# cleinc/bts

Hardware: NVIDIA H100
Metric: training images/sec (352x704, DenseNet-161) (higher is better)
Workload: dtype f32

## Files before the change

bts_b200/csrc/wgmma_tf32.cuh:

```cuda
#pragma once
#include <stdint.h>

namespace tc {

template <int N> struct Wgmma;

template <> struct Wgmma<16> {
    static __device__ __forceinline__ void mma(float (&d)[8], uint64_t a, uint64_t b, uint32_t scale_d) {
        asm volatile(
            "{\n\t.reg .pred p;\n\tsetp.ne.b32 p, %10, 0;\n\t"
            "wgmma.mma_async.sync.aligned.m64n16k8.f32.tf32.tf32 {%0, %1, %2, %3, %4, %5, %6, %7}, %8, %9, p, 1, 1;\n\t}"
            : "+f"(d[0]), "+f"(d[1]), "+f"(d[2]), "+f"(d[3]), "+f"(d[4]), "+f"(d[5]), "+f"(d[6]), "+f"(d[7])
            : "l"(a), "l"(b), "r"(scale_d));
    }
    static __device__ __forceinline__ void mma_rs(float (&d)[8], const uint32_t (&a)[4], uint64_t b, uint32_t scale_d) {
        asm volatile(
            "{\n\t.reg .pred p;\n\tsetp.ne.b32 p, %13, 0;\n\t"
            "wgmma.mma_async.sync.aligned.m64n16k8.f32.tf32.tf32 {%0, %1, %2, %3, %4, %5, %6, %7}, {%8, %9, %10, %11}, %12, p, 1, 1;\n\t}"
            : "+f"(d[0]), "+f"(d[1]), "+f"(d[2]), "+f"(d[3]), "+f"(d[4]), "+f"(d[5]), "+f"(d[6]), "+f"(d[7])
            : "r"(a[0]), "r"(a[1]), "r"(a[2]), "r"(a[3]), "l"(b), "r"(scale_d));
    }
};

template <> struct Wgmma<32> {
    static __device__ __forceinline__ void mma(float (&d)[16], uint64_t a, uint64_t b, uint32_t scale_d) {
        asm volatile(
            "{\n\t.reg .pred p;\n\tsetp.ne.b32 p, %18, 0;\n\t"
            "wgmma.mma_async.sync.aligned.m64n32k8.f32.tf32.tf32 {%0, %1, %2, %3, %4, %5, %6, %7, %8, %9, %10, %11, %12, %13, %14, %15}, %16, %17, p, 1, 1;\n\t}"
            : "+f"(d[0]), "+f"(d[1]), "+f"(d[2]), "+f"(d[3]), "+f"(d[4]), "+f"(d[5]), "+f"(d[6]), "+f"(d[7]), "+f"(d[8]), "+f"(d[9]), "+f"(d[10]), "+f"(d[11]), "+f"(d[12]), "+f"(d[13]), "+f"(d[14]), "+f"(d[15])
            : "l"(a), "l"(b), "r"(scale_d));
    }
    static __device__ __forceinline__ void mma_rs(float (&d)[16], const uint32_t (&a)[4], uint64_t b, uint32_t scale_d) {
        asm volatile(
            "{\n\t.reg .pred p;\n\tsetp.ne.b32 p, %21, 0;\n\t"
            "wgmma.mma_async.sync.aligned.m64n32k8.f32.tf32.tf32 {%0, %1, %2, %3, %4, %5, %6, %7, %8, %9, %10, %11, %12, %13, %14, %15}, {%16, %17, %18, %19}, %20, p, 1, 1;\n\t}"
            : "+f"(d[0]), "+f"(d[1]), "+f"(d[2]), "+f"(d[3]), "+f"(d[4]), "+f"(d[5]), "+f"(d[6]), "+f"(d[7]), "+f"(d[8]), "+f"(d[9]), "+f"(d[10]), "+f"(d[11]), "+f"(d[12]), "+f"(d[13]), "+f"(d[14]), "+f"(d[15])
            : "r"(a[0]), "r"(a[1]), "r"(a[2]), "r"(a[3]), "l"(b), "r"(scale_d));
    }
};

template <> struct Wgmma<48> {
    static __device__ __forceinline__ void mma(float (&d)[24], uint64_t a, uint64_t b, uint32_t scale_d) {
        asm volatile(
            "{\n\t.reg .pred p;\n\tsetp.ne.b32 p, %26, 0;\n\t"
            "wgmma.mma_async.sync.aligned.m64n48k8.f32.tf32.tf32 {%0, %1, %2, %3, %4, %5, %6, %7, %8, %9, %10, %11, %12, %13, %14, %15, %16, %17, %18, %19, %20, %21, %22, %23}, %24, %25, p, 1, 1;\n\t}"
            : "+f"(d[0]), "+f"(d[1]), "+f"(d[2]), "+f"(d[3]), "+f"(d[4]), "+f"(d[5]), "+f"(d[6]), "+f"(d[7]), "+f"(d[8]), "+f"(d[9]), "+f"(d[10]), "+f"(d[11]), "+f"(d[12]), "+f"(d[13]), "+f"(d[14]), "+f"(d[15]), "+f"(d[16]), "+f"(d[17]), "+f"(d[18]), "+f"(d[19]), "+f"(d[20]), "+f"(d[21]), "+f"(d[22]), "+f"(d[23])
            : "l"(a), "l"(b), "r"(scale_d));
    }
    static __device__ __forceinline__ void mma_rs(float (&d)[24], const uint32_t (&a)[4], uint64_t b, uint32_t scale_d) {
        asm volatile(
            "{\n\t.reg .pred p;\n\tsetp.ne.b32 p, %29, 0;\n\t"
            "wgmma.mma_async.sync.aligned.m64n48k8.f32.tf32.tf32 {%0, %1, %2, %3, %4, %5, %6, %7, %8, %9, %10, %11, %12, %13, %14, %15, %16, %17, %18, %19, %20, %21, %22, %23}, {%24, %25, %26, %27}, %28, p, 1, 1;\n\t}"
            : "+f"(d[0]), "+f"(d[1]), "+f"(d[2]), "+f"(d[3]), "+f"(d[4]), "+f"(d[5]), "+f"(d[6]), "+f"(d[7]), "+f"(d[8]), "+f"(d[9]), "+f"(d[10]), "+f"(d[11]), "+f"(d[12]), "+f"(d[13]), "+f"(d[14]), "+f"(d[15]), "+f"(d[16]), "+f"(d[17]), "+f"(d[18]), "+f"(d[19]), "+f"(d[20]), "+f"(d[21]), "+f"(d[22]), "+f"(d[23])
            : "r"(a[0]), "r"(a[1]), "r"(a[2]), "r"(a[3]), "l"(b), "r"(scale_d));
    }
};

template <> struct Wgmma<64> {
    static __device__ __forceinline__ void mma(float (&d)[32], uint64_t a, uint64_t b, uint32_t scale_d) {
        asm volatile(
            "{\n\t.reg .pred p;\n\tsetp.ne.b32 p, %34, 0;\n\t"
            "wgmma.mma_async.sync.aligned.m64n64k8.f32.tf32.tf32 {%0, %1, %2, %3, %4, %5, %6, %7, %8, %9, %10, %11, %12, %13, %14, %15, %16, %17, %18, %19, %20, %21, %22, %23, %24, %25, %26, %27, %28, %29, %30, %31}, %32, %33, p, 1, 1;\n\t}"
            : "+f"(d[0]), "+f"(d[1]), "+f"(d[2]), "+f"(d[3]), "+f"(d[4]), "+f"(d[5]), "+f"(d[6]), "+f"(d[7]), "+f"(d[8]), "+f"(d[9]), "+f"(d[10]), "+f"(d[11]), "+f"(d[12]), "+f"(d[13]), "+f"(d[14]), "+f"(d[15]), "+f"(d[16]), "+f"(d[17]), "+f"(d[18]), "+f"(d[19]), "+f"(d[20]), "+f"(d[21]), "+f"(d[22]), "+f"(d[23]), "+f"(d[24]), "+f"(d[25]), "+f"(d[26]), "+f"(d[27]), "+f"(d[28]), "+f"(d[29]), "+f"(d[30]), "+f"(d[31])
            : "l"(a), "l"(b), "r"(scale_d));
    }
    static __device__ __forceinline__ void mma_rs(float (&d)[32], const uint32_t (&a)[4], uint64_t b, uint32_t scale_d) {
        asm volatile(
            "{\n\t.reg .pred p;\n\tsetp.ne.b32 p, %37, 0;\n\t"
            "wgmma.mma_async.sync.aligned.m64n64k8.f32.tf32.tf32 {%0, %1, %2, %3, %4, %5, %6, %7, %8, %9, %10, %11, %12, %13, %14, %15, %16, %17, %18, %19, %20, %21, %22, %23, %24, %25, %26, %27, %28, %29, %30, %31}, {%32, %33, %34, %35}, %36, p, 1, 1;\n\t}"
            : "+f"(d[0]), "+f"(d[1]), "+f"(d[2]), "+f"(d[3]), "+f"(d[4]), "+f"(d[5]), "+f"(d[6]), "+f"(d[7]), "+f"(d[8]), "+f"(d[9]), "+f"(d[10]), "+f"(d[11]), "+f"(d[12]), "+f"(d[13]), "+f"(d[14]), "+f"(d[15]), "+f"(d[16]), "+f"(d[17]), "+f"(d[18]), "+f"(d[19]), "+f"(d[20]), "+f"(d[21]), "+f"(d[22]), "+f"(d[23]), "+f"(d[24]), "+f"(d[25]), "+f"(d[26]), "+f"(d[27]), "+f"(d[28]), "+f"(d[29]), "+f"(d[30]), "+f"(d[31])
            : "r"(a[0]), "r"(a[1]), "r"(a[2]), "r"(a[3]), "l"(b), "r"(scale_d));
    }
};

template <> struct Wgmma<80> {
    static __device__ __forceinline__ void mma(float (&d)[40], uint64_t a, uint64_t b, uint32_t scale_d) {
        asm volatile(
            "{\n\t.reg .pred p;\n\tsetp.ne.b32 p, %42, 0;\n\t"
            "wgmma.mma_async.sync.aligned.m64n80k8.f32.tf32.tf32 {%0, %1, %2, %3, %4, %5, %6, %7, %8, %9, %10, %11, %12, %13, %14, %15, %16, %17, %18, %19, %20, %21, %22, %23, %24, %25, %26, %27, %28, %29, %30, %31, %32, %33, %34, %35, %36, %37, %38, %39}, %40, %41, p, 1, 1;\n\t}"
            : "+f"(d[0]), "+f"(d[1]), "+f"(d[2]), "+f"(d[3]), "+f"(d[4]), "+f"(d[5]), "+f"(d[6]), "+f"(d[7]), "+f"(d[8]), "+f"(d[9]), "+f"(d[10]), "+f"(d[11]), "+f"(d[12]), "+f"(d[13]), "+f"(d[14]), "+f"(d[15]), "+f"(d[16]), "+f"(d[17]), "+f"(d[18]), "+f"(d[19]), "+f"(d[20]), "+f"(d[21]), "+f"(d[22]), "+f"(d[23]), "+f"(d[24]), "+f"(d[25]), "+f"(d[26]), "+f"(d[27]), "+f"(d[28]), "+f"(d[29]), "+f"(d[30]), "+f"(d[31]), "+f"(d[32]), "+f"(d[33]), "+f"(d[34]), "+f"(d[35]), "+f"(d[36]), "+f"(d[37]), "+f"(d[38]), "+f"(d[39])
            : "l"(a), "l"(b), "r"(scale_d));
    }
};

}
```

bts_b200/csrc/wgrad2_tc.cu:

```cuda
#include <cuda.h>

#include <cstring>
#include <type_traits>

#include "tc_common.cuh"

using namespace tc;

namespace {

constexpr int BLOCK_CI = 64;
constexpr int X_CHUNKS = BLOCK_CI / 32;
constexpr int KP = 16;
constexpr uint32_t CORE_SBO = 4 * 128 + 16;
constexpr int A_BYTES = BLOCK_CI / 8 * CORE_SBO;
constexpr int MAX_TAPS = 9;
constexpr int MAX_NT = 144;
constexpr int MAX_STAGES = 4;
constexpr int CONSUMER_THREADS = 256;
constexpr int LOADER_WARP = CONSUMER_THREADS / 32;
constexpr int GROUPS = 3;
constexpr int PRODUCERS = 128 * GROUPS;
constexpr int NUM_THREADS = CONSUMER_THREADS + 32 + PRODUCERS;
constexpr int SMEM_BUDGET = 224 * 1024;
constexpr int MAX_RING = 4;
constexpr int X_RAW_BYTES = KP * BLOCK_CI * 4;

struct W2Params {
    const float *x; long long xs;
    int B, Hs, Ws, up, Cin;
    int KH, KW, pad, dil;
    const float *pre_scale, *pre_shift;
    const float *dy; long long dys;
    int Cout, Hout, Wout, Hin, Win;
    int cg, nb;
    int nchunks;
    float *part;
    int splitK, kb_per_split, KBq;
    int Mq;
    int stages, stage_bytes, precision;
    int ring, slot_bytes, seg_bytes, segw, tox_max, slot_tx;
};

template <int PRE, bool UP, bool VEC, bool TMA>
__global__ void __launch_bounds__(NUM_THREADS, 1) wgrad2_tc_kernel(const W2Params p, const __grid_constant__ CUtensorMap tmx,
                                                                   const __grid_constant__ CUtensorMap tmd) {
    extern __shared__ __align__(1024) uint8_t smem_raw[];
    const uint32_t base = (smem_u32(smem_raw) + 1023u) & ~1023u;
    uint8_t *sm = smem_raw + (base - smem_u32(smem_raw));
    const int taps = p.KH * p.KW;
    const int S = p.stages;
    const uint32_t ring_off = (uint32_t)S * (uint32_t)p.stage_bytes;
    const uint32_t pre_off = ring_off + (TMA ? (uint32_t)p.ring * (uint32_t)p.slot_bytes : 0u);
    float *s_scale = reinterpret_cast<float *>(sm + pre_off);
    float *s_shift = s_scale + BLOCK_CI;
    const uint32_t bar0 = base + pre_off + 2 * BLOCK_CI * 4;
    auto full = [&](int s) { return bar0 + 8u * s; };
    auto empty = [&](int s) { return bar0 + 8u * (MAX_STAGES + s); };
    auto rfull = [&](int j) { return bar0 + 8u * (2 * MAX_STAGES + j); };
    auto rempty = [&](int j) { return bar0 + 8u * (2 * MAX_STAGES + MAX_RING + j); };
    const int warp = threadIdx.x >> 5, lane = threadIdx.x & 31;
    const int ci_tile = blockIdx.x, cgi = blockIdx.y, split = blockIdx.z;
    const int co0 = cgi * p.cg;
    const int ncol = min(p.cg, ((p.Cout - co0 + 15) >> 4) << 4);
    const int nb = p.nb;
    const int n_total = taps * ncol;
    const uint32_t b_half = (uint32_t)p.nchunks * 4u * CORE_SBO;
    const int kb0 = split * p.kb_per_split;
    int kb1 = kb0 + p.kb_per_split;
    if (kb1 > p.KBq) kb1 = p.KBq;
    const int nkb = kb1 > kb0 ? kb1 - kb0 : 0;

    if (threadIdx.x == 0) {
        for (int s = 0; s < MAX_STAGES; ++s) {
            mbar_init(full(s), PRODUCERS);
            mbar_init(empty(s), CONSUMER_THREADS);
        }
        for (int j = 0; j < MAX_RING; ++j) {
            mbar_init(rfull(j), 1);
            mbar_init(rempty(j), PRODUCERS);
        }
        asm volatile("fence.mbarrier_init.release.cluster;" ::: "memory");
    }
    if (PRE >= 2) {
        for (int c = threadIdx.x; c < BLOCK_CI; c += NUM_THREADS) {
            const int ch = ci_tile * BLOCK_CI + c;
            s_scale[c] = ch < p.Cin ? p.pre_scale[ch] : 0.f;
            s_shift[c] = ch < p.Cin ? p.pre_shift[ch] : 0.f;
        }
    }
    for (int i = threadIdx.x; i < S * p.stage_bytes / 16; i += NUM_THREADS) st_shared_v4(base + i * 16, 0.f, 0.f, 0.f, 0.f);
    fence_proxy_async();
    __syncthreads();

    if (warp == LOADER_WARP) {
        if (TMA && lane == 0) {
            if (!UP) tma_prefetch_desc(&tmx);
            tma_prefetch_desc(&tmd);
            int j = 0;
            uint32_t ph = 0;
            for (int it = 0; it < nkb; ++it) {
                mbar_wait(rempty(j), ph ^ 1);
                const uint32_t dst = base + ring_off + (uint32_t)j * (uint32_t)p.slot_bytes;
                const int q0 = (kb0 + it) * KP;
                mbar_arrive_expect_tx(rfull(j), (uint32_t)p.slot_tx);
                uint32_t seg = dst;
                if (!UP) {
                    tma_tile_2d(dst, &tmx, ci_tile * BLOCK_CI, q0, rfull(j));
                    seg += X_RAW_BYTES;
                }
                for (int ky = 0; ky < p.KH; ++ky)
                    tma_tile_2d(seg + (uint32_t)ky * (uint32_t)p.seg_bytes, &tmd, co0,
                                q0 - (ky * p.dil - p.pad) * p.Wout - p.tox_max, rfull(j));
                if (++j == p.ring) { j = 0; ph ^= 1; }
            }
        }
    } else if (warp < LOADER_WARP) {
        const int wg = warp >> 2;
        const int n_half = (n_total + 31) / 32 * 16;
        const int n0 = wg ? n_half : 0, n_mine = wg ? n_total - n_half : n_half;
        auto consume = [&](auto NT) {
            constexpr int N = decltype(NT)::value;
            float acc[N > 0 ? N / 2 : 1];
#pragma unroll
            for (int i = 0; i < (N > 0 ? N / 2 : 1); ++i) acc[i] = 0.f;
            const bool single = p.precision != 0;
            int s = 0;
            uint32_t ph = 0;
            for (int it = 0; it < nkb; ++it) {
                mbar_wait(full(s), ph);
                wgmma_fence();
                const uint32_t a_hi = base + (uint32_t)s * (uint32_t)p.stage_bytes, a_lo = a_hi + A_BYTES;
                const uint32_t b_hi = a_hi + 2 * A_BYTES + (uint32_t)(n0 >> 3) * CORE_SBO, b_lo = b_hi + b_half;
                if constexpr (N > 0) {
#pragma unroll
                    for (int kg = 0; kg < KP / 8; ++kg) {
                        const uint32_t ko = (uint32_t)kg * 256u;
                        const uint64_t dah = make_desc_core(a_hi + ko, 128, CORE_SBO), dal = make_desc_core(a_lo + ko, 128, CORE_SBO);
                        const uint64_t dbh = make_desc_core(b_hi + ko, 128, CORE_SBO), dbl = make_desc_core(b_lo + ko, 128, CORE_SBO);
                        const uint32_t accumulate = (it | kg) != 0;
                        if (single) {
                            Wgmma<N>::mma(acc, dah, dbh, accumulate);
                        } else {
                            Wgmma<N>::mma(acc, dal, dbh, accumulate);
                            Wgmma<N>::mma(acc, dah, dbl, 1);
                            Wgmma<N>::mma(acc, dah, dbh, 1);
                        }
                    }
                }
                wgmma_commit();
                wgmma_wait<0>();
                mbar_arrive(empty(s));
                if (++s == S) { s = 0; ph ^= 1; }
            }
            wgmma_wait<0>();
            wgmma_fence_operands(acc);
            if (N == 0) return;
            const bool ovec = (p.Cout & 1) == 0 && ((((uintptr_t)p.part) & 7) == 0) && ((co0 & 1) == 0);
#pragma unroll
            for (int i = 0; i < 2; ++i) {
                const int ci = ci_tile * BLOCK_CI + (warp & 3) * 16 + (lane >> 2) + 8 * i;
                if (ci >= p.Cin) continue;
#pragma unroll
                for (int j = 0; j < (N > 0 ? N / 8 : 0); ++j) {
                    const int n = n0 + 8 * j + (lane & 3) * 2;
                    if (n >= n0 + n_mine) continue;
                    const int t = n / ncol, cc = n - t * ncol;
                    float *dst = p.part + (((long long)split * taps + t) * p.Cin + ci) * p.Cout + co0 + cc;
                    const float v0 = acc[4 * j + 2 * i], v1 = acc[4 * j + 2 * i + 1];
                    if (ovec && co0 + cc + 1 < p.Cout) {
                        *reinterpret_cast<float2 *>(dst) = make_float2(v0, v1);
                    } else {
                        if (co0 + cc < p.Cout) dst[0] = v0;
                        if (co0 + cc + 1 < p.Cout) dst[1] = v1;
                    }
                }
            }
        };
        switch (n_mine) {
            case 0: consume(std::integral_constant<int, 0>()); break;
            case 16: consume(std::integral_constant<int, 16>()); break;
            case 32: consume(std::integral_constant<int, 32>()); break;
            case 48: consume(std::integral_constant<int, 48>()); break;
            case 64: consume(std::integral_constant<int, 64>()); break;
            default: consume(std::integral_constant<int, 80>()); break;
        }
    } else {
        const int pt = threadIdx.x - (CONSUMER_THREADS + 32);
        const int unit = pt & 7;
        const int row = (pt >> 3) & 15;
        const int half = pt >> 7;
        const bool xq = half < X_CHUNKS;
        constexpr bool AFF = PRE >= 2;
        constexpr bool RELU = (PRE & 1) != 0;
        auto core_off = [&](int n) {
            return (uint32_t)(n >> 3) * CORE_SBO + (uint32_t)(row >> 2) * 128u + (uint32_t)(n & 7) * 16u + (uint32_t)(row & 3) * 4u;
        };
        const int xs = (int)p.xs, dys = (int)p.dys;
        const int cbx = ci_tile * BLOCK_CI + half * 32 + unit * 4;
        const int cbd = co0 + unit * 4;
        const float *__restrict__ xg = p.x;
        const float *__restrict__ dg = p.dy;
        float sc[1][4], sh[1][4];
        if (AFF) {
#pragma unroll
            for (int e = 0; e < 4; ++e) {
                sc[0][e] = xq ? s_scale[half * 32 + unit * 4 + e] : 0.f;
                sh[0][e] = xq ? s_shift[half * 32 + unit * 4 + e] : 0.f;
            }
        }
        int qx, qy, qb;
        {
            const int q = kb0 * KP + row;
            qx = q % p.Win;
            const int r = q / p.Win;
            qy = r % p.Hin;
            qb = r / p.Hin;
        }
        constexpr int NBU = 6;
        constexpr int NAU = 1;
        const bool single = taps == 1;
        auto unit_tap = [&](int j) { return single ? 0 : half + GROUPS * j; };
        auto unit_chunk = [&](int j, int ch) { return single ? half + GROUPS * (2 * j + ch) : ch; };
        int toy[NBU / 2], tox[NBU / 2], tky[NBU / 2];
#pragma unroll
        for (int j = 0; j < NBU / 2; ++j) {
            const int t = unit_tap(j);
            const int ky = t / p.KW, kx = t - ky * p.KW;
            toy[j] = ky * p.dil - p.pad;
            tox[j] = kx * p.dil - p.pad;
            tky[j] = ky < p.KH ? ky : 0;
        }
        uint32_t boff[NBU];
        bool blive[NBU];
#pragma unroll
        for (int j = 0; j < NBU / 2; ++j)
#pragma unroll
            for (int ch = 0; ch < 2; ++ch) {
                const int t = unit_tap(j), cc = unit_chunk(j, ch);
                const int c = unit * 4 + cc * 32;
                const int n = t * ncol + c;
                blive[j * 2 + ch] = t < taps && cc < nb && c < ncol;
                boff[j * 2 + ch] = core_off(n);
            }
        struct Cursor { int qx, qy, qb; };
        Cursor cur = {qx, qy, qb};
        auto advance = [&](Cursor &c) {
            c.qx += KP;
            while (c.qx >= p.Win) {
                c.qx -= p.Win;
                if (++c.qy == p.Hin) { c.qy = 0; ++c.qb; }
            }
        };
        auto load_x = [&](int it, const Cursor &c_, F4(&va)[NAU], bool &okx) {
            const int q = (kb0 + it) * KP + row;
            okx = q < p.Mq;
            const int sy = UP ? (c_.qy >> 1) : c_.qy, sx = UP ? (c_.qx >> 1) : c_.qx;
            const int xoff = ((c_.qb * p.Hs + sy) * p.Ws + sx) * xs;
#pragma unroll
            for (int ch = 0; ch < NAU; ++ch) {
                const int c = cbx + ch * 32;
                const bool live = xq && okx && c < p.Cin;
                if (VEC) {
                    float4 v = make_float4(0.f, 0.f, 0.f, 0.f);
                    if (live) v = __ldg(reinterpret_cast<const float4 *>(xg + xoff + c));
                    if (c + 3 >= p.Cin) {
                        if (c + 1 >= p.Cin) v.y = 0.f;
                        if (c + 2 >= p.Cin) v.z = 0.f;
                        v.w = 0.f;
                    }
                    va[ch].v[0] = v.x; va[ch].v[1] = v.y; va[ch].v[2] = v.z; va[ch].v[3] = v.w;
                } else {
#pragma unroll
                    for (int e = 0; e < 4; ++e) {
                        float v = 0.f;
                        if (live && c + e < p.Cin) v = __ldg(xg + xoff + c + e);
                        va[ch].v[e] = v;
                    }
                }
            }
        };
        auto load_d = [&](const Cursor &c_, bool okx, F4(&vb)[NBU]) {
#pragma unroll
            for (int j = 0; j < NBU / 2; ++j) {
                const int t = unit_tap(j);
                const int py = c_.qy - toy[j], px = c_.qx - tox[j];
                const bool okd = okx && t < taps && (unsigned)py < (unsigned)p.Hout && (unsigned)px < (unsigned)p.Wout;
                const int doff = ((c_.qb * p.Hout + py) * p.Wout + px) * dys;
#pragma unroll
                for (int ch = 0; ch < 2; ++ch) {
                    const int c = cbd + unit_chunk(j, ch) * 32;
                    const bool live = okd && blive[j * 2 + ch] && c < p.Cout;
                    F4 &dst = vb[j * 2 + ch];
                    if (VEC) {
                        float4 v = make_float4(0.f, 0.f, 0.f, 0.f);
                        if (live) v = __ldg(reinterpret_cast<const float4 *>(dg + doff + c));
                        if (c + 3 >= p.Cout) {
                            if (c + 1 >= p.Cout) v.y = 0.f;
                            if (c + 2 >= p.Cout) v.z = 0.f;
                            v.w = 0.f;
                        }
                        dst.v[0] = v.x; dst.v[1] = v.y; dst.v[2] = v.z; dst.v[3] = v.w;
                    } else {
#pragma unroll
                        for (int e = 0; e < 4; ++e) {
                            float v = 0.f;
                            if (live && c + e < p.Cout) v = __ldg(dg + doff + c + e);
                            dst.v[e] = v;
                        }
                    }
                }
            }
        };
        auto load = [&](int it, F4(&va)[NAU], F4(&vb)[NBU], bool &okx) {
            load_x(it, cur, va, okx);
            load_d(cur, okx, vb);
            advance(cur);
        };
        auto ring_read = [&](int it, uint32_t slot, F4(&va)[NAU], F4(&vb)[NBU], bool &okx) {
            const int q = (kb0 + it) * KP + row;
            okx = q < p.Mq;
            uint32_t segb = slot;
            if (!UP) {
                float4 v = make_float4(0.f, 0.f, 0.f, 0.f);
                if (xq) v = ld_shared_v4(slot + (uint32_t)((row * BLOCK_CI + half * 32 + unit * 4) * 4));
                va[0].v[0] = v.x; va[0].v[1] = v.y; va[0].v[2] = v.z; va[0].v[3] = v.w;
                segb += X_RAW_BYTES;
            }
#pragma unroll
            for (int j = 0; j < NBU / 2; ++j) {
                const int t = unit_tap(j);
                const int py = cur.qy - toy[j], px = cur.qx - tox[j];
                const bool okd = okx && t < taps && (unsigned)py < (unsigned)p.Hout && (unsigned)px < (unsigned)p.Wout;
                const uint32_t rowb = segb + (uint32_t)tky[j] * (uint32_t)p.seg_bytes +
                                      (uint32_t)((row + p.tox_max - tox[j]) * p.cg + unit * 4) * 4u;
#pragma unroll
                for (int ch = 0; ch < 2; ++ch) {
                    F4 &dst = vb[j * 2 + ch];
                    float4 v = make_float4(0.f, 0.f, 0.f, 0.f);
                    if (okd && blive[j * 2 + ch]) v = ld_shared_v4(rowb + (uint32_t)unit_chunk(j, ch) * 128u);
                    dst.v[0] = v.x; dst.v[1] = v.y; dst.v[2] = v.z; dst.v[3] = v.w;
                }
            }
            advance(cur);
        };
        auto split_store = [&](uint32_t hi_addr, uint32_t lo_addr, const F4 &v) {
            float hi[4], lo[4];
#pragma unroll
            for (int e = 0; e < 4; ++e) split_tf32(v.v[e], hi[e], lo[e]);
#pragma unroll
            for (int e = 0; e < 4; ++e) {
                st_shared_f32(hi_addr + 16u * e, hi[e]);
                st_shared_f32(lo_addr + 16u * e, lo[e]);
            }
        };
        int st_s = 0;
        uint32_t st_ph = 0;
        auto store = [&](int it, F4(&va)[NAU], F4(&vb)[NBU], bool okx) {
            const int s = st_s;
            const uint32_t ph = st_ph;
            if (++st_s == S) { st_s = 0; st_ph ^= 1; }
            if (PRE != 0) {
#pragma unroll
                for (int ch = 0; ch < NAU; ++ch)
#pragma unroll
                    for (int e = 0; e < 4; ++e) {
                        float a = va[ch].v[e];
                        if (AFF) {
                            a = fmaf(a, sc[ch][e], sh[ch][e]);
                            if (RELU) a = fmaxf(a, 0.f);
                            a = okx ? a : 0.f;
                        } else {
                            a = fmaxf(a, 0.f);
                        }
                        va[ch].v[e] = a;
                    }
            }
            mbar_wait(empty(s), ph ^ 1);
            const uint32_t a_hi = base + (uint32_t)s * (uint32_t)p.stage_bytes, a_lo = a_hi + A_BYTES;
            const uint32_t b_hi = a_hi + 2 * A_BYTES, b_lo = b_hi + b_half;
            if (xq) {
                const uint32_t o = core_off(half * 32 + unit * 4);
                split_store(a_hi + o, a_lo + o, va[0]);
            }
#pragma unroll
            for (int j = 0; j < NBU; ++j)
                if (blive[j]) split_store(b_hi + boff[j], b_lo + boff[j], vb[j]);
            fence_proxy_async();
            mbar_arrive(full(s));
        };
        if constexpr (!TMA) {
            F4 a0[NAU], a1[NAU], b0[NBU], b1[NBU];
            bool k0 = false, k1 = false;
            int it = 0;
            if (it < nkb) load(it, a0, b0, k0);
            for (; it < nkb; it += 2) {
                const bool more = it + 1 < nkb;
                if (more) load(it + 1, a1, b1, k1);
                store(it, a0, b0, k0);
                if (more) {
                    if (it + 2 < nkb) load(it + 2, a0, b0, k0);
                    store(it + 1, a1, b1, k1);
                }
            }
        } else {
            F4 xc[NAU], xn[NAU], va[NAU], vb[NBU];
            bool kc = false, kn = false, okx = false;
            Cursor pre = cur;
            if (UP && nkb > 0) { load_x(0, pre, xc, kc); advance(pre); }
            int rj = 0;
            uint32_t rph = 0;
            for (int it = 0; it < nkb; ++it) {
                if (UP && it + 1 < nkb) { load_x(it + 1, pre, xn, kn); advance(pre); }
                mbar_wait(rfull(rj), rph);
                ring_read(it, base + ring_off + (uint32_t)rj * (uint32_t)p.slot_bytes, va, vb, okx);
                mbar_arrive(rempty(rj));
                if (++rj == p.ring) { rj = 0; rph ^= 1; }
                if (UP) {
                    store(it, xc, vb, okx);
#pragma unroll
                    for (int ch = 0; ch < NAU; ++ch) xc[ch] = xn[ch];
                    kc = kn;
                } else {
                    store(it, va, vb, okx);
                }
            }
        }
    }
}

}

int bts_wgrad2_cg(int Cout, int taps) {
    int cap = (MAX_NT / taps) / 16 * 16;
    if (taps == 1) {
        if (cap > 128) cap = 128;
    } else if (cap > 48) {
        cap = 48;
    }
    if (cap < 16) return 0;
    const int groups = (Cout + cap - 1) / cap;
    int cg = ((Cout + groups - 1) / groups + 15) / 16 * 16;
    if (cg > cap) cg = cap;
    return cg;
}

static long long g_w2_min_pixels = 12000;
static int g_w2_pointwise = 1;
extern "C" int bts_wgrad2_set_pointwise(int on) { g_w2_pointwise = on ? 1 : 0; return 0; }
static int g_w2_min_kb = 8;
extern "C" int bts_wgrad2_set_min_pixels(long long n) { g_w2_min_pixels = n < 0 ? 12000 : n; return 0; }
extern "C" int bts_wgrad2_set_min_kblocks(int n) { g_w2_min_kb = n < 1 ? 8 : n; return 0; }

bool bts_wgrad2_eligible(int Cout, int KH, int KW, int stride, long long Mq) {
    const int taps = KH * KW;
    if (stride != 1 || Mq < g_w2_min_pixels || taps > MAX_TAPS || bts_wgrad2_cg(Cout, taps) <= 0) return false;
    if (taps == 1) return g_w2_pointwise && Cout > 64 && Cout <= 256;
    return Cout <= 64;
}

void bts_wgrad2_plan(int B, int Hin, int Win, int Cin, int Cout, int KH, int KW, int *splitK) {
    const int taps = KH * KW;
    const int cg = bts_wgrad2_cg(Cout, taps);
    const long long Mq = (long long)B * Hin * Win;
    const long long KBq = (Mq + KP - 1) / KP;
    const long long tiles = (long long)((Cin + BLOCK_CI - 1) / BLOCK_CI) * ((Cout + cg - 1) / cg);
    const int sms = bts_num_sms();
    long long max_split = (KBq + g_w2_min_kb - 1) / g_w2_min_kb;
    if (max_split < 1) max_split = 1;
    if (max_split > 512) max_split = 512;
    long long split = 1;
    double best = -1.0;
    for (long long sp = 1; sp <= max_split; ++sp) {
        const long long ctas = tiles * sp;
        const long long waves = (ctas + sms - 1) / sms;
        if (waves > 2 && sp > 1) break;
        const double eff = (double)ctas / (double)(waves * sms);
        if (eff > best + 1e-9) { best = eff; split = sp; }
    }
    *splitK = (int)split;
}

typedef CUresult (*EncodeTiledFn)(CUtensorMap *, CUtensorMapDataType, cuuint32_t, void *, const cuuint64_t *, const cuuint64_t *,
                                  const cuuint32_t *, const cuuint32_t *, CUtensorMapInterleave, CUtensorMapSwizzle,
                                  CUtensorMapL2promotion, CUtensorMapFloatOOBfill);

static EncodeTiledFn encode_tiled_fn() {
    static EncodeTiledFn fn = nullptr;
    static bool tried = false;
    if (!tried) {
        tried = true;
        void *ptr = nullptr;
        cudaDriverEntryPointQueryResult qres;
        if (cudaGetDriverEntryPoint("cuTensorMapEncodeTiled", &ptr, cudaEnableDefault, &qres) == cudaSuccess &&
            qres == cudaDriverEntryPointSuccess)
            fn = reinterpret_cast<EncodeTiledFn>(ptr);
    }
    return fn;
}

static bool make_rows_map(CUtensorMap *map, const float *base, long long pixel_stride, int channels, long long pixels, int box_c,
                          int box_p) {
    EncodeTiledFn fn = encode_tiled_fn();
    if (!fn || box_c > 256 || box_p > 256) return false;
    const cuuint64_t gdim[2] = {(cuuint64_t)channels, (cuuint64_t)pixels};
    const cuuint64_t gstr[1] = {(cuuint64_t)pixel_stride * 4};
    const cuuint32_t box[2] = {(cuuint32_t)box_c, (cuuint32_t)box_p};
    const cuuint32_t estr[2] = {1, 1};
    return fn(map, CU_TENSOR_MAP_DATA_TYPE_FLOAT32, 2, const_cast<float *>(base), gdim, gstr, box, estr,
              CU_TENSOR_MAP_INTERLEAVE_NONE, CU_TENSOR_MAP_SWIZZLE_NONE, CU_TENSOR_MAP_L2_PROMOTION_L2_128B,
              CU_TENSOR_MAP_FLOAT_OOB_FILL_NONE) == CUDA_SUCCESS;
}

static int g_w2_tma = 1;
extern "C" int bts_wgrad2_set_tma(int on) { g_w2_tma = on ? 1 : 0; return 0; }

int bts_wgrad2_launch(const float *x, long long xs, int B, int Hs, int Ws, int up, int Cin, int KH, int KW, int pad,
                      int dil, const float *pre_scale, const float *pre_shift, int pre_relu, const float *dy,
                      long long dys, int Cout, int Hout, int Wout, float *workspace, int splitK, int precision,
                      cudaStream_t st) {
    W2Params p;
    const int taps = KH * KW;
    p.x = x; p.xs = xs; p.B = B; p.Hs = Hs; p.Ws = Ws; p.up = up; p.Cin = Cin;
    p.KH = KH; p.KW = KW; p.pad = pad; p.dil = dil;
    p.pre_scale = pre_scale; p.pre_shift = pre_shift;
    p.dy = dy; p.dys = dys; p.Cout = Cout; p.Hout = Hout; p.Wout = Wout;
    p.Hin = up ? 2 * Hs : Hs; p.Win = up ? 2 * Ws : Ws;
    p.cg = bts_wgrad2_cg(Cout, taps);
    p.nb = (p.cg + 31) / 32;
    p.part = workspace; p.splitK = splitK;
    const long long Mq = (long long)B * p.Hin * p.Win;
    if (Mq > 0x7ffffff0LL) return BTS_EINVAL;
    p.Mq = (int)Mq;
    p.KBq = (int)((Mq + KP - 1) / KP);
    p.kb_per_split = (p.KBq + splitK - 1) / splitK;
    p.nchunks = (taps * p.cg + 31) / 32;
    p.stage_bytes = 2 * A_BYTES + 2 * p.nchunks * 4 * (int)CORE_SBO;
    p.stages = SMEM_BUDGET / p.stage_bytes;
    if (p.stages > MAX_STAGES) p.stages = MAX_STAGES;
    if (p.stages < 2) return BTS_EINVAL;
    p.precision = precision;
    const int pre = (pre_scale ? 2 : 0) | (pre_relu ? 1 : 0);
    const bool vec = bts_aligned16(x) && (xs % 4 == 0) && bts_aligned16(dy) && (dys % 4 == 0);
    CUtensorMap tmx, tmd;
    memset(&tmx, 0, sizeof(tmx));
    memset(&tmd, 0, sizeof(tmd));
    bool tma = false;
    p.ring = p.slot_bytes = p.seg_bytes = p.segw = p.tox_max = p.slot_tx = 0;
    if (g_w2_tma && vec && KH <= 3 && Hout == p.Hin && Wout == p.Win) {
        p.segw = KP + (KW - 1) * dil;
        p.tox_max = (KW - 1) * dil - pad;
        p.seg_bytes = (p.segw * p.cg * 4 + 127) / 128 * 128;
        p.slot_bytes = (up ? 0 : X_RAW_BYTES) + KH * p.seg_bytes;
        p.slot_tx = (up ? 0 : X_RAW_BYTES) + KH * p.segw * p.cg * 4;
        int st_try = p.stages > 3 ? 3 : p.stages;
        for (; st_try >= 2 && !tma; --st_try) {
            const int ring = (SMEM_BUDGET - st_try * p.stage_bytes) / p.slot_bytes;
            if (ring >= 3 || (st_try == 2 && ring >= 2)) {
                p.stages = st_try;
                p.ring = ring > MAX_RING ? MAX_RING : ring;
                tma = true;
            }
        }
        if (tma && p.segw <= 256)
            tma = make_rows_map(&tmd, dy, dys, Cout, (long long)B * Hout * Wout, p.cg, p.segw) &&
                  (up || make_rows_map(&tmx, x, xs, Cin, Mq, BLOCK_CI, KP));
        else
            tma = false;
        if (!tma) {
            p.ring = 0;
            p.stages = SMEM_BUDGET / p.stage_bytes > MAX_STAGES ? MAX_STAGES : SMEM_BUDGET / p.stage_bytes;
        }
    }
    const int smem = p.stages * p.stage_bytes + p.ring * p.slot_bytes + 2 * BLOCK_CI * 4 + 256 + 1024;
    dim3 grid((Cin + BLOCK_CI - 1) / BLOCK_CI, (Cout + p.cg - 1) / p.cg, splitK);
    cudaError_t err = cudaSuccess;
#define BTS_LAUNCH(PRE, UP, VEC, TMA)                                                                                 \
    do {                                                                                                              \
        static int attr_smem_[BTS_MAX_DEVICES] = {}; int &attr_smem = attr_smem_[bts_cur_device()];                   \
        if (attr_smem < smem) {                                                                                       \
            err = cudaFuncSetAttribute(wgrad2_tc_kernel<PRE, UP, VEC, TMA>, cudaFuncAttributeMaxDynamicSharedMemorySize, \
                                       SMEM_BUDGET + 2 * BLOCK_CI * 4 + 256 + 1024);                                  \
            if (err != cudaSuccess) return (int)err;                                                                  \
            attr_smem = SMEM_BUDGET + 2 * BLOCK_CI * 4 + 256 + 1024;                                                  \
        }                                                                                                             \
        wgrad2_tc_kernel<PRE, UP, VEC, TMA><<<grid, NUM_THREADS, smem, st>>>(p, tmx, tmd);                            \
    } while (0)
#define BTS_DISPATCH_UV(PRE)                                                                     \
    do {                                                                                         \
        if (tma) { if (p.up) BTS_LAUNCH(PRE, true, true, true); else BTS_LAUNCH(PRE, false, true, true); } \
        else if (p.up) { if (vec) BTS_LAUNCH(PRE, true, true, false); else BTS_LAUNCH(PRE, true, false, false); }   \
        else { if (vec) BTS_LAUNCH(PRE, false, true, false); else BTS_LAUNCH(PRE, false, false, false); }      \
    } while (0)
    switch (pre) {
        case 0: BTS_DISPATCH_UV(0); break;
        case 1: BTS_DISPATCH_UV(1); break;
        case 2: BTS_DISPATCH_UV(2); break;
        default: BTS_DISPATCH_UV(3); break;
    }
#undef BTS_DISPATCH_UV
#undef BTS_LAUNCH
    BTS_LAUNCH_CHECK();
    return 0;
}
```

Before: 69.20.

## Feed wgrad A operand from registers and double the K depth per stage

Rewrites the weight-gradient TF32 kernel so the A operand (activations) is stored raw in a swizzled smem tile, loaded and split into hi/lo TF32 parts by the consumer warps, and passed to register-sourced wgmma instead of smem descriptors. K per stage doubles from 16 to 32 pixels, the dedicated TMA loader warp is removed and its issue logic moved into producer thread 0, and the producer layout is reorganised to 256 threads with per-chunk precomputed offsets. Split-K granularity is now decoupled from KP via a 16-pixel split unit. This aims to halve A-side split/store work and smem traffic for A, at the cost of more consumer register pressure and a serialised commit/wait per stage.

```diff
diff --git a/bts_b200/csrc/wgmma_tf32.cuh b/bts_b200/csrc/wgmma_tf32.cuh
--- a/bts_b200/csrc/wgmma_tf32.cuh
+++ b/bts_b200/csrc/wgmma_tf32.cuh
@@ -6,13 +6,6 @@
 template <int N> struct Wgmma;
 
 template <> struct Wgmma<16> {
-    static __device__ __forceinline__ void mma(float (&d)[8], uint64_t a, uint64_t b, uint32_t scale_d) {
-        asm volatile(
-            "{\n\t.reg .pred p;\n\tsetp.ne.b32 p, %10, 0;\n\t"
-            "wgmma.mma_async.sync.aligned.m64n16k8.f32.tf32.tf32 {%0, %1, %2, %3, %4, %5, %6, %7}, %8, %9, p, 1, 1;\n\t}"
-            : "+f"(d[0]), "+f"(d[1]), "+f"(d[2]), "+f"(d[3]), "+f"(d[4]), "+f"(d[5]), "+f"(d[6]), "+f"(d[7])
-            : "l"(a), "l"(b), "r"(scale_d));
-    }
     static __device__ __forceinline__ void mma_rs(float (&d)[8], const uint32_t (&a)[4], uint64_t b, uint32_t scale_d) {
         asm volatile(
             "{\n\t.reg .pred p;\n\tsetp.ne.b32 p, %13, 0;\n\t"
@@ -23,13 +16,6 @@
 };
 
 template <> struct Wgmma<32> {
-    static __device__ __forceinline__ void mma(float (&d)[16], uint64_t a, uint64_t b, uint32_t scale_d) {
-        asm volatile(
-            "{\n\t.reg .pred p;\n\tsetp.ne.b32 p, %18, 0;\n\t"
-            "wgmma.mma_async.sync.aligned.m64n32k8.f32.tf32.tf32 {%0, %1, %2, %3, %4, %5, %6, %7, %8, %9, %10, %11, %12, %13, %14, %15}, %16, %17, p, 1, 1;\n\t}"
-            : "+f"(d[0]), "+f"(d[1]), "+f"(d[2]), "+f"(d[3]), "+f"(d[4]), "+f"(d[5]), "+f"(d[6]), "+f"(d[7]), "+f"(d[8]), "+f"(d[9]), "+f"(d[10]), "+f"(d[11]), "+f"(d[12]), "+f"(d[13]), "+f"(d[14]), "+f"(d[15])
-            : "l"(a), "l"(b), "r"(scale_d));
-    }
     static __device__ __forceinline__ void mma_rs(float (&d)[16], const uint32_t (&a)[4], uint64_t b, uint32_t scale_d) {
         asm volatile(
             "{\n\t.reg .pred p;\n\tsetp.ne.b32 p, %21, 0;\n\t"
@@ -40,13 +26,6 @@
 };
 
 template <> struct Wgmma<48> {
-    static __device__ __forceinline__ void mma(float (&d)[24], uint64_t a, uint64_t b, uint32_t scale_d) {
-        asm volatile(
-            "{\n\t.reg .pred p;\n\tsetp.ne.b32 p, %26, 0;\n\t"
-            "wgmma.mma_async.sync.aligned.m64n48k8.f32.tf32.tf32 {%0, %1, %2, %3, %4, %5, %6, %7, %8, %9, %10, %11, %12, %13, %14, %15, %16, %17, %18, %19, %20, %21, %22, %23}, %24, %25, p, 1, 1;\n\t}"
-            : "+f"(d[0]), "+f"(d[1]), "+f"(d[2]), "+f"(d[3]), "+f"(d[4]), "+f"(d[5]), "+f"(d[6]), "+f"(d[7]), "+f"(d[8]), "+f"(d[9]), "+f"(d[10]), "+f"(d[11]), "+f"(d[12]), "+f"(d[13]), "+f"(d[14]), "+f"(d[15]), "+f"(d[16]), "+f"(d[17]), "+f"(d[18]), "+f"(d[19]), "+f"(d[20]), "+f"(d[21]), "+f"(d[22]), "+f"(d[23])
-            : "l"(a), "l"(b), "r"(scale_d));
-    }
     static __device__ __forceinline__ void mma_rs(float (&d)[24], const uint32_t (&a)[4], uint64_t b, uint32_t scale_d) {
         asm volatile(
             "{\n\t.reg .pred p;\n\tsetp.ne.b32 p, %29, 0;\n\t"
@@ -57,13 +36,6 @@
 };
 
 template <> struct Wgmma<64> {
-    static __device__ __forceinline__ void mma(float (&d)[32], uint64_t a, uint64_t b, uint32_t scale_d) {
-        asm volatile(
-            "{\n\t.reg .pred p;\n\tsetp.ne.b32 p, %34, 0;\n\t"
-            "wgmma.mma_async.sync.aligned.m64n64k8.f32.tf32.tf32 {%0, %1, %2, %3, %4, %5, %6, %7, %8, %9, %10, %11, %12, %13, %14, %15, %16, %17, %18, %19, %20, %21, %22, %23, %24, %25, %26, %27, %28, %29, %30, %31}, %32, %33, p, 1, 1;\n\t}"
-            : "+f"(d[0]), "+f"(d[1]), "+f"(d[2]), "+f"(d[3]), "+f"(d[4]), "+f"(d[5]), "+f"(d[6]), "+f"(d[7]), "+f"(d[8]), "+f"(d[9]), "+f"(d[10]), "+f"(d[11]), "+f"(d[12]), "+f"(d[13]), "+f"(d[14]), "+f"(d[15]), "+f"(d[16]), "+f"(d[17]), "+f"(d[18]), "+f"(d[19]), "+f"(d[20]), "+f"(d[21]), "+f"(d[22]), "+f"(d[23]), "+f"(d[24]), "+f"(d[25]), "+f"(d[26]), "+f"(d[27]), "+f"(d[28]), "+f"(d[29]), "+f"(d[30]), "+f"(d[31])
-            : "l"(a), "l"(b), "r"(scale_d));
-    }
     static __device__ __forceinline__ void mma_rs(float (&d)[32], const uint32_t (&a)[4], uint64_t b, uint32_t scale_d) {
         asm volatile(
             "{\n\t.reg .pred p;\n\tsetp.ne.b32 p, %37, 0;\n\t"
@@ -74,12 +46,12 @@
 };
 
 template <> struct Wgmma<80> {
-    static __device__ __forceinline__ void mma(float (&d)[40], uint64_t a, uint64_t b, uint32_t scale_d) {
+    static __device__ __forceinline__ void mma_rs(float (&d)[40], const uint32_t (&a)[4], uint64_t b, uint32_t scale_d) {
         asm volatile(
-            "{\n\t.reg .pred p;\n\tsetp.ne.b32 p, %42, 0;\n\t"
-            "wgmma.mma_async.sync.aligned.m64n80k8.f32.tf32.tf32 {%0, %1, %2, %3, %4, %5, %6, %7, %8, %9, %10, %11, %12, %13, %14, %15, %16, %17, %18, %19, %20, %21, %22, %23, %24, %25, %26, %27, %28, %29, %30, %31, %32, %33, %34, %35, %36, %37, %38, %39}, %40, %41, p, 1, 1;\n\t}"
+            "{\n\t.reg .pred p;\n\tsetp.ne.b32 p, %45, 0;\n\t"
+            "wgmma.mma_async.sync.aligned.m64n80k8.f32.tf32.tf32 {%0, %1, %2, %3, %4, %5, %6, %7, %8, %9, %10, %11, %12, %13, %14, %15, %16, %17, %18, %19, %20, %21, %22, %23, %24, %25, %26, %27, %28, %29, %30, %31, %32, %33, %34, %35, %36, %37, %38, %39}, {%40, %41, %42, %43}, %44, p, 1, 1;\n\t}"
             : "+f"(d[0]), "+f"(d[1]), "+f"(d[2]), "+f"(d[3]), "+f"(d[4]), "+f"(d[5]), "+f"(d[6]), "+f"(d[7]), "+f"(d[8]), "+f"(d[9]), "+f"(d[10]), "+f"(d[11]), "+f"(d[12]), "+f"(d[13]), "+f"(d[14]), "+f"(d[15]), "+f"(d[16]), "+f"(d[17]), "+f"(d[18]), "+f"(d[19]), "+f"(d[20]), "+f"(d[21]), "+f"(d[22]), "+f"(d[23]), "+f"(d[24]), "+f"(d[25]), "+f"(d[26]), "+f"(d[27]), "+f"(d[28]), "+f"(d[29]), "+f"(d[30]), "+f"(d[31]), "+f"(d[32]), "+f"(d[33]), "+f"(d[34]), "+f"(d[35]), "+f"(d[36]), "+f"(d[37]), "+f"(d[38]), "+f"(d[39])
-            : "l"(a), "l"(b), "r"(scale_d));
+            : "r"(a[0]), "r"(a[1]), "r"(a[2]), "r"(a[3]), "l"(b), "r"(scale_d));
     }
 };
 
diff --git a/bts_b200/csrc/wgrad2_tc.cu b/bts_b200/csrc/wgrad2_tc.cu
--- a/bts_b200/csrc/wgrad2_tc.cu
+++ b/bts_b200/csrc/wgrad2_tc.cu
@@ -10,21 +10,20 @@
 namespace {
 
 constexpr int BLOCK_CI = 64;
-constexpr int X_CHUNKS = BLOCK_CI / 32;
-constexpr int KP = 16;
-constexpr uint32_t CORE_SBO = 4 * 128 + 16;
-constexpr int A_BYTES = BLOCK_CI / 8 * CORE_SBO;
+constexpr int KP = 32;
+constexpr int SPLIT_PX = 16;
+constexpr uint32_t CORE_SBO = KP / 4 * 128 + 16;
+constexpr int X_ROW_BYTES = BLOCK_CI * 4;
+constexpr int X_BYTES = KP * X_ROW_BYTES;
 constexpr int MAX_TAPS = 9;
 constexpr int MAX_NT = 144;
+constexpr int MAX_CHUNKS = (MAX_NT + 31) / 32;
 constexpr int MAX_STAGES = 4;
 constexpr int CONSUMER_THREADS = 256;
-constexpr int LOADER_WARP = CONSUMER_THREADS / 32;
-constexpr int GROUPS = 3;
-constexpr int PRODUCERS = 128 * GROUPS;
-constexpr int NUM_THREADS = CONSUMER_THREADS + 32 + PRODUCERS;
+constexpr int PRODUCERS = 256;
+constexpr int NUM_THREADS = CONSUMER_THREADS + PRODUCERS;
 constexpr int SMEM_BUDGET = 224 * 1024;
 constexpr int MAX_RING = 4;
-constexpr int X_RAW_BYTES = KP * BLOCK_CI * 4;
 
 struct W2Params {
     const float *x; long long xs;
@@ -33,12 +32,11 @@
     const float *pre_scale, *pre_shift;
     const float *dy; long long dys;
     int Cout, Hout, Wout, Hin, Win;
-    int cg, nb;
-    int nchunks;
+    int cg;
     float *part;
-    int splitK, kb_per_split, KBq;
+    int splitK, px_per_split;
     int Mq;
-    int stages, stage_bytes, precision;
+    int stages, stage_bytes, b_half, precision;
     int ring, slot_bytes, seg_bytes, segw, tox_max, slot_tx;
 };
 
@@ -50,7 +48,8 @@
     uint8_t *sm = smem_raw + (base - smem_u32(smem_raw));
     const int taps = p.KH * p.KW;
     const int S = p.stages;
-    const uint32_t ring_off = (uint32_t)S * (uint32_t)p.stage_bytes;
+    const uint32_t stage_bytes = (uint32_t)p.stage_bytes;
+    const uint32_t ring_off = (uint32_t)S * stage_bytes;
     const uint32_t pre_off = ring_off + (TMA ? (uint32_t)p.ring * (uint32_t)p.slot_bytes : 0u);
     float *s_scale = reinterpret_cast<float *>(sm + pre_off);
     float *s_shift = s_scale + BLOCK_CI;
@@ -63,13 +62,10 @@
     const int ci_tile = blockIdx.x, cgi = blockIdx.y, split = blockIdx.z;
     const int co0 = cgi * p.cg;
     const int ncol = min(p.cg, ((p.Cout - co0 + 15) >> 4) << 4);
-    const int nb = p.nb;
     const int n_total = taps * ncol;
-    const uint32_t b_half = (uint32_t)p.nchunks * 4u * CORE_SBO;
-    const int kb0 = split * p.kb_per_split;
-    int kb1 = kb0 + p.kb_per_split;
-    if (kb1 > p.KBq) kb1 = p.KBq;
-    const int nkb = kb1 > kb0 ? kb1 - kb0 : 0;
+    const int q_begin = split * p.px_per_split;
+    const int q_end = min(q_begin + p.px_per_split, p.Mq);
+    const int nkb = q_end > q_begin ? (q_end - q_begin + KP - 1) / KP : 0;
 
     if (threadIdx.x == 0) {
         for (int s = 0; s < MAX_STAGES; ++s) {
@@ -89,72 +85,66 @@
             s_shift[c] = ch < p.Cin ? p.pre_shift[ch] : 0.f;
         }
     }
-    for (int i = threadIdx.x; i < S * p.stage_bytes / 16; i += NUM_THREADS) st_shared_v4(base + i * 16, 0.f, 0.f, 0.f, 0.f);
-    fence_proxy_async();
     __syncthreads();
 
-    if (warp == LOADER_WARP) {
-        if (TMA && lane == 0) {
-            if (!UP) tma_prefetch_desc(&tmx);
-            tma_prefetch_desc(&tmd);
-            int j = 0;
-            uint32_t ph = 0;
-            for (int it = 0; it < nkb; ++it) {
-                mbar_wait(rempty(j), ph ^ 1);
-                const uint32_t dst = base + ring_off + (uint32_t)j * (uint32_t)p.slot_bytes;
-                const int q0 = (kb0 + it) * KP;
-                mbar_arrive_expect_tx(rfull(j), (uint32_t)p.slot_tx);
-                uint32_t seg = dst;
-                if (!UP) {
-                    tma_tile_2d(dst, &tmx, ci_tile * BLOCK_CI, q0, rfull(j));
-                    seg += X_RAW_BYTES;
-                }
-                for (int ky = 0; ky < p.KH; ++ky)
-                    tma_tile_2d(seg + (uint32_t)ky * (uint32_t)p.seg_bytes, &tmd, co0,
-                                q0 - (ky * p.dil - p.pad) * p.Wout - p.tox_max, rfull(j));
-                if (++j == p.ring) { j = 0; ph ^= 1; }
-            }
-        }
-    } else if (warp < LOADER_WARP) {
+    if (warp < CONSUMER_THREADS / 32) {
         const int wg = warp >> 2;
         const int n_half = (n_total + 31) / 32 * 16;
         const int n0 = wg ? n_half : 0, n_mine = wg ? n_total - n_half : n_half;
+        const int q = lane & 3;
+        const int c = (warp & 3) * 16 + (lane >> 2);
+        const uint32_t aF = (uint32_t)q * X_ROW_BYTES + ((uint32_t)((c >> 2) ^ (2 * q)) << 4) + (uint32_t)(c & 3) * 4u;
+        const bool single = p.precision != 0;
         auto consume = [&](auto NT) {
             constexpr int N = decltype(NT)::value;
             float acc[N > 0 ? N / 2 : 1];
 #pragma unroll
             for (int i = 0; i < (N > 0 ? N / 2 : 1); ++i) acc[i] = 0.f;
-            const bool single = p.precision != 0;
             int s = 0;
             uint32_t ph = 0;
             for (int it = 0; it < nkb; ++it) {
                 mbar_wait(full(s), ph);
-                wgmma_fence();
-                const uint32_t a_hi = base + (uint32_t)s * (uint32_t)p.stage_bytes, a_lo = a_hi + A_BYTES;
-                const uint32_t b_hi = a_hi + 2 * A_BYTES + (uint32_t)(n0 >> 3) * CORE_SBO, b_lo = b_hi + b_half;
                 if constexpr (N > 0) {
-#pragma unroll
-                    for (int kg = 0; kg < KP / 8; ++kg) {
-                        const uint32_t ko = (uint32_t)kg * 256u;
-                        const uint64_t dah = make_desc_core(a_hi + ko, 128, CORE_SBO), dal = make_desc_core(a_lo + ko, 128, CORE_SBO);
+                    const uint32_t st = base + (uint32_t)s * stage_bytes;
+                    uint32_t hi[KP / 8][4], lo[KP / 8][4];
+#pragma unroll
+                    for (int k = 0; k < KP / 8; ++k) {
+#pragma unroll
+                        for (int j = 0; j < 4; ++j) {
+                            const uint32_t x = ld_shared_u32(st + (aF ^ (32u * (j & 1))) + (uint32_t)(8 * k + 4 * (j >> 1)) * X_ROW_BYTES);
+                            float h, l;
+                            split_tf32(__uint_as_float(x), h, l);
+                            hi[k][j] = __float_as_uint(h);
+                            lo[k][j] = __float_as_uint(l);
+                        }
+                    }
+                    const uint32_t b_hi = st + X_BYTES + (uint32_t)(n0 >> 3) * CORE_SBO, b_lo = b_hi + (uint32_t)p.b_half;
+                    wgmma_fence();
+#pragma unroll
+                    for (int k = 0; k < KP / 8; ++k) {
+                        const uint32_t ko = (uint32_t)k * 256u;
                         const uint64_t dbh = make_desc_core(b_hi + ko, 128, CORE_SBO), dbl = make_desc_core(b_lo + ko, 128, CORE_SBO);
-                        const uint32_t accumulate = (it | kg) != 0;
+                        const uint32_t accumulate = (it | k) != 0;
                         if (single) {
-                            Wgmma<N>::mma(acc, dah, dbh, accumulate);
+                            Wgmma<N>::mma_rs(acc, hi[k], dbh, accumulate);
                         } else {
-                            Wgmma<N>::mma(acc, dal, dbh, accumulate);
-                            Wgmma<N>::mma(acc, dah, dbl, 1);
-                            Wgmma<N>::mma(acc, dah, dbh, 1);
+                            Wgmma<N>::mma_rs(acc, lo[k], dbh, accumulate);
+                            Wgmma<N>::mma_rs(acc, hi[k], dbl, 1);
+                            Wgmma<N>::mma_rs(acc, hi[k], dbh, 1);
                         }
                     }
-                }
-                wgmma_commit();
-                wgmma_wait<0>();
+                    wgmma_commit();
+                    wgmma_wait<0>();
+                    wgmma_fence_operands(acc);
+#pragma unroll
+                    for (int k = 0; k < KP / 8; ++k) {
+                        wgmma_fence_operands(hi[k]);
+                        wgmma_fence_operands(lo[k]);
+                    }
+                }
                 mbar_arrive(empty(s));
                 if (++s == S) { s = 0; ph ^= 1; }
             }
-            wgmma_wait<0>();
-            wgmma_fence_operands(acc);
             if (N == 0) return;
             const bool ovec = (p.Cout & 1) == 0 && ((((uintptr_t)p.part) & 7) == 0) && ((co0 & 1) == 0);
 #pragma unroll
@@ -186,65 +176,53 @@
             default: consume(std::integral_constant<int, 80>()); break;
         }
     } else {
-        const int pt = threadIdx.x - (CONSUMER_THREADS + 32);
-        const int unit = pt & 7;
-        const int row = (pt >> 3) & 15;
-        const int half = pt >> 7;
-        const bool xq = half < X_CHUNKS;
+        const int pt = threadIdx.x - CONSUMER_THREADS;
+        const int ul = pt & 7;
+        const int row = pt >> 3;
         constexpr bool AFF = PRE >= 2;
         constexpr bool RELU = (PRE & 1) != 0;
+        const uint32_t xoff = (uint32_t)row * X_ROW_BYTES + ((uint32_t)(ul ^ (2 * (row & 3))) << 4);
         auto core_off = [&](int n) {
             return (uint32_t)(n >> 3) * CORE_SBO + (uint32_t)(row >> 2) * 128u + (uint32_t)(n & 7) * 16u + (uint32_t)(row & 3) * 4u;
         };
         const int xs = (int)p.xs, dys = (int)p.dys;
-        const int cbx = ci_tile * BLOCK_CI + half * 32 + unit * 4;
-        const int cbd = co0 + unit * 4;
+        const int cbx = ci_tile * BLOCK_CI + ul * 4;
         const float *__restrict__ xg = p.x;
         const float *__restrict__ dg = p.dy;
-        float sc[1][4], sh[1][4];
+        float sc[2][4], sh[2][4];
         if (AFF) {
 #pragma unroll
-            for (int e = 0; e < 4; ++e) {
-                sc[0][e] = xq ? s_scale[half * 32 + unit * 4 + e] : 0.f;
-                sh[0][e] = xq ? s_shift[half * 32 + unit * 4 + e] : 0.f;
-            }
-        }
-        int qx, qy, qb;
+            for (int h = 0; h < 2; ++h)
+#pragma unroll
+                for (int e = 0; e < 4; ++e) {
+                    sc[h][e] = s_scale[h * 32 + ul * 4 + e];
+                    sh[h][e] = s_shift[h * 32 + ul * 4 + e];
+                }
+        }
+        int toy[MAX_CHUNKS], tox[MAX_CHUNKS], ucol[MAX_CHUNKS];
+        uint32_t boff[MAX_CHUNKS], roff[MAX_CHUNKS];
+        bool blive[MAX_CHUNKS];
+#pragma unroll
+        for (int ch = 0; ch < MAX_CHUNKS; ++ch) {
+            const int n = ch * 32 + ul * 4;
+            blive[ch] = n < n_total;
+            const int t = blive[ch] ? n / ncol : 0;
+            const int ky = t / p.KW, kx = t - ky * p.KW;
+            toy[ch] = ky * p.dil - p.pad;
+            tox[ch] = kx * p.dil - p.pad;
+            ucol[ch] = n - t * ncol;
+            boff[ch] = core_off(n);
+            roff[ch] = (uint32_t)ky * (uint32_t)p.seg_bytes + (uint32_t)((row + p.tox_max - tox[ch]) * p.cg + ucol[ch]) * 4u;
+        }
+        struct Cursor { int qx, qy, qb; };
+        Cursor cur;
         {
-            const int q = kb0 * KP + row;
-            qx = q % p.Win;
+            const int q = q_begin + row;
+            cur.qx = q % p.Win;
             const int r = q / p.Win;
-            qy = r % p.Hin;
-            qb = r / p.Hin;
-        }
-        constexpr int NBU = 6;
-        constexpr int NAU = 1;
-        const bool single = taps == 1;
-        auto unit_tap = [&](int j) { return single ? 0 : half + GROUPS * j; };
-        auto unit_chunk = [&](int j, int ch) { return single ? half + GROUPS * (2 * j + ch) : ch; };
-        int toy[NBU / 2], tox[NBU / 2], tky[NBU / 2];
-#pragma unroll
-        for (int j = 0; j < NBU / 2; ++j) {
-            const int t = unit_tap(j);
-            const int ky = t / p.KW, kx = t - ky * p.KW;
-            toy[j] = ky * p.dil - p.pad;
-            tox[j] = kx * p.dil - p.pad;
-            tky[j] = ky < p.KH ? ky : 0;
-        }
-        uint32_t boff[NBU];
-        bool blive[NBU];
-#pragma unroll
-        for (int j = 0; j < NBU / 2; ++j)
-#pragma unroll
-            for (int ch = 0; ch < 2; ++ch) {
-                const int t = unit_tap(j), cc = unit_chunk(j, ch);
-                const int c = unit * 4 + cc * 32;
-                const int n = t * ncol + c;
-                blive[j * 2 + ch] = t < taps && cc < nb && c < ncol;
-                boff[j * 2 + ch] = core_off(n);
-            }
-        struct Cursor { int qx, qy, qb; };
-        Cursor cur = {qx, qy, qb};
+            cur.qy = r % p.Hin;
+            cur.qb = r / p.Hin;
+        }
         auto advance = [&](Cursor &c) {
             c.qx += KP;
             while (c.qx >= p.Win) {
@@ -252,159 +230,158 @@
                 if (++c.qy == p.Hin) { c.qy = 0; ++c.qb; }
             }
         };
-        auto load_x = [&](int it, const Cursor &c_, F4(&va)[NAU], bool &okx) {
-            const int q = (kb0 + it) * KP + row;
-            okx = q < p.Mq;
+        auto pixel_ok = [&](int it) { return q_begin + it * KP + row < q_end; };
+        auto load_x = [&](int it, const Cursor &c_, F4(&va)[2], bool &okx) {
+            okx = pixel_ok(it);
             const int sy = UP ? (c_.qy >> 1) : c_.qy, sx = UP ? (c_.qx >> 1) : c_.qx;
-            const int xoff = ((c_.qb * p.Hs + sy) * p.Ws + sx) * xs;
-#pragma unroll
-            for (int ch = 0; ch < NAU; ++ch) {
-                const int c = cbx + ch * 32;
-                const bool live = xq && okx && c < p.Cin;
+            const int xo = ((c_.qb * p.Hs + sy) * p.Ws + sx) * xs;
+#pragma unroll
+            for (int h = 0; h < 2; ++h) {
+                const int c = cbx + h * 32;
+                const bool live = okx && c < p.Cin;
                 if (VEC) {
                     float4 v = make_float4(0.f, 0.f, 0.f, 0.f);
-                    if (live) v = __ldg(reinterpret_cast<const float4 *>(xg + xoff + c));
+                    if (live) v = __ldg(reinterpret_cast<const float4 *>(xg + xo + c));
                     if (c + 3 >= p.Cin) {
                         if (c + 1 >= p.Cin) v.y = 0.f;
                         if (c + 2 >= p.Cin) v.z = 0.f;
                         v.w = 0.f;
                     }
-                    va[ch].v[0] = v.x; va[ch].v[1] = v.y; va[ch].v[2] = v.z; va[ch].v[3] = v.w;
+                    va[h].v[0] = v.x; va[h].v[1] = v.y; va[h].v[2] = v.z; va[h].v[3] = v.w;
                 } else {
 #pragma unroll
                     for (int e = 0; e < 4; ++e) {
                         float v = 0.f;
-                        if (live && c + e < p.Cin) v = __ldg(xg + xoff + c + e);
-                        va[ch].v[e] = v;
-                    }
-                }
-            }
-        };
-        auto load_d = [&](const Cursor &c_, bool okx, F4(&vb)[NBU]) {
-#pragma unroll
-            for (int j = 0; j < NBU / 2; ++j) {
-                const int t = unit_tap(j);
-                const int py = c_.qy - toy[j], px = c_.qx - tox[j];
-                const bool okd = okx && t < taps && (unsigned)py < (unsigned)p.Hout && (unsigned)px < (unsigned)p.Wout;
+                        if (live && c + e < p.Cin) v = __ldg(xg + xo + c + e);
+                        va[h].v[e] = v;
+                    }
+                }
+            }
+        };
+        auto load_d = [&](const Cursor &c_, bool okx, F4(&vb)[MAX_CHUNKS]) {
+#pragma unroll
+            for (int ch = 0; ch < MAX_CHUNKS; ++ch) {
+                const int py = c_.qy - toy[ch], px = c_.qx - tox[ch];
+                const bool okd = okx && blive[ch] && (unsigned)py < (unsigned)p.Hout && (unsigned)px < (unsigned)p.Wout;
                 const int doff = ((c_.qb * p.Hout + py) * p.Wout + px) * dys;
-#pragma unroll
-                for (int ch = 0; ch < 2; ++ch) {
-                    const int c = cbd + unit_chunk(j, ch) * 32;
-                    const bool live = okd && blive[j * 2 + ch] && c < p.Cout;
-                    F4 &dst = vb[j * 2 + ch];
-                    if (VEC) {
-                        float4 v = make_float4(0.f, 0.f, 0.f, 0.f);
-                        if (live) v = __ldg(reinterpret_cast<const float4 *>(dg + doff + c));
-                        if (c + 3 >= p.Cout) {
-                            if (c + 1 >= p.Cout) v.y = 0.f;
-                            if (c + 2 >= p.Cout) v.z = 0.f;
-                            v.w = 0.f;
-                        }
-                        dst.v[0] = v.x; dst.v[1] = v.y; dst.v[2] = v.z; dst.v[3] = v.w;
-                    } else {
-#pragma unroll
-                        for (int e = 0; e < 4; ++e) {
-                            float v = 0.f;
-                            if (live && c + e < p.Cout) v = __ldg(dg + doff + c + e);
-                            dst.v[e] = v;
-                        }
-                    }
-                }
-            }
-        };
-        auto load = [&](int it, F4(&va)[NAU], F4(&vb)[NBU], bool &okx) {
+                const int c = co0 + ucol[ch];
+                const bool live = okd && c < p.Cout;
+                F4 &dst = vb[ch];
+                if (VEC) {
+                    float4 v = make_float4(0.f, 0.f, 0.f, 0.f);
+                    if (live) v = __ldg(reinterpret_cast<const float4 *>(dg + doff + c));
+                    if (c + 3 >= p.Cout) {
+                        if (c + 1 >= p.Cout) v.y = 0.f;
+                        if (c + 2 >= p.Cout) v.z = 0.f;
+                        v.w = 0.f;
+                    }
+                    dst.v[0] = v.x; dst.v[1] = v.y; dst.v[2] = v.z; dst.v[3] = v.w;
+                } else {
+#pragma unroll
+                    for (int e = 0; e < 4; ++e) {
+                        float v = 0.f;
+                        if (live && c + e < p.Cout) v = __ldg(dg + doff + c + e);
+                        dst.v[e] = v;
+                    }
+                }
+            }
+        };
+        auto load = [&](int it, F4(&va)[2], F4(&vb)[MAX_CHUNKS], bool &okx) {
             load_x(it, cur, va, okx);
             load_d(cur, okx, vb);
             advance(cur);
         };
-        auto ring_read = [&](int it, uint32_t slot, F4(&va)[NAU], F4(&vb)[NBU], bool &okx) {
-            const int q = (kb0 + it) * KP + row;
-            okx = q < p.Mq;
+        auto ring_read = [&](int it, uint32_t slot, F4(&va)[2], F4(&vb)[MAX_CHUNKS], bool &okx) {
+            okx = pixel_ok(it);
             uint32_t segb = slot;
             if (!UP) {
+#pragma unroll
+                for (int h = 0; h < 2; ++h) {
+                    const float4 v = ld_shared_v4(slot + (uint32_t)(row * X_ROW_BYTES + (h * 32 + ul * 4) * 4));
+                    va[h].v[0] = v.x; va[h].v[1] = v.y; va[h].v[2] = v.z; va[h].v[3] = v.w;
+                }
+                segb += X_BYTES;
+            }
+#pragma unroll
+            for (int ch = 0; ch < MAX_CHUNKS; ++ch) {
+                const int py = cur.qy - toy[ch], px = cur.qx - tox[ch];
+                const bool okd = okx && blive[ch] && (unsigned)py < (unsigned)p.Hout && (unsigned)px < (unsigned)p.Wout;
                 float4 v = make_float4(0.f, 0.f, 0.f, 0.f);
-                if (xq) v = ld_shared_v4(slot + (uint32_t)((row * BLOCK_CI + half * 32 + unit * 4) * 4));
-                va[0].v[0] = v.x; va[0].v[1] = v.y; va[0].v[2] = v.z; va[0].v[3] = v.w;
-                segb += X_RAW_BYTES;
-            }
-#pragma unroll
-            for (int j = 0; j < NBU / 2; ++j) {
-                const int t = unit_tap(j);
-                const int py = cur.qy - toy[j], px = cur.qx - tox[j];
-                const bool okd = okx && t < taps && (unsigned)py < (unsigned)p.Hout && (unsigned)px < (unsigned)p.Wout;
-                const uint32_t rowb = segb + (uint32_t)tky[j] * (uint32_t)p.seg_bytes +
-                                      (uint32_t)((row + p.tox_max - tox[j]) * p.cg + unit * 4) * 4u;
-#pragma unroll
-                for (int ch = 0; ch < 2; ++ch) {
-                    F4 &dst = vb[j * 2 + ch];
-                    float4 v = make_float4(0.f, 0.f, 0.f, 0.f);
-                    if (okd && blive[j * 2 + ch]) v = ld_shared_v4(rowb + (uint32_t)unit_chunk(j, ch) * 128u);
-                    dst.v[0] = v.x; dst.v[1] = v.y; dst.v[2] = v.z; dst.v[3] = v.w;
-                }
+                if (okd) v = ld_shared_v4(segb + roff[ch]);
+                vb[ch].v[0] = v.x; vb[ch].v[1] = v.y; vb[ch].v[2] = v.z; vb[ch].v[3] = v.w;
             }
             advance(cur);
-        };
-        auto split_store = [&](uint32_t hi_addr, uint32_t lo_addr, const F4 &v) {
-            float hi[4], lo[4];
-#pragma unroll
-            for (int e = 0; e < 4; ++e) split_tf32(v.v[e], hi[e], lo[e]);
-#pragma unroll
-            for (int e = 0; e < 4; ++e) {
-                st_shared_f32(hi_addr + 16u * e, hi[e]);
-                st_shared_f32(lo_addr + 16u * e, lo[e]);
-            }
         };
         int st_s = 0;
         uint32_t st_ph = 0;
-        auto store = [&](int it, F4(&va)[NAU], F4(&vb)[NBU], bool okx) {
+        auto store = [&](F4(&va)[2], F4(&vb)[MAX_CHUNKS], bool okx) {
             const int s = st_s;
             const uint32_t ph = st_ph;
             if (++st_s == S) { st_s = 0; st_ph ^= 1; }
-            if (PRE != 0) {
-#pragma unroll
-                for (int ch = 0; ch < NAU; ++ch)
-#pragma unroll
-                    for (int e = 0; e < 4; ++e) {
-                        float a = va[ch].v[e];
-                        if (AFF) {
-                            a = fmaf(a, sc[ch][e], sh[ch][e]);
-                            if (RELU) a = fmaxf(a, 0.f);
-                            a = okx ? a : 0.f;
-                        } else {
-                            a = fmaxf(a, 0.f);
-                        }
-                        va[ch].v[e] = a;
-                    }
-            }
+#pragma unroll
+            for (int h = 0; h < 2; ++h)
+#pragma unroll
+                for (int e = 0; e < 4; ++e) {
+                    float a = va[h].v[e];
+                    if (AFF) a = fmaf(a, sc[h][e], sh[h][e]);
+                    if (RELU) a = fmaxf(a, 0.f);
+                    va[h].v[e] = okx ? a : 0.f;
+                }
             mbar_wait(empty(s), ph ^ 1);
-            const uint32_t a_hi = base + (uint32_t)s * (uint32_t)p.stage_bytes, a_lo = a_hi + A_BYTES;
-            const uint32_t b_hi = a_hi + 2 * A_BYTES, b_lo = b_hi + b_half;
-            if (xq) {
-                const uint32_t o = core_off(half * 32 + unit * 4);
-                split_store(a_hi + o, a_lo + o, va[0]);
-            }
-#pragma unroll
-            for (int j = 0; j < NBU; ++j)
-                if (blive[j]) split_store(b_hi + boff[j], b_lo + boff[j], vb[j]);
+            const uint32_t st = base + (uint32_t)s * stage_bytes;
+#pragma unroll
+            for (int h = 0; h < 2; ++h)
+                st_shared_v4(st + xoff + 128u * h, va[h].v[0], va[h].v[1], va[h].v[2], va[h].v[3]);
+            const uint32_t b_hi = st + X_BYTES, b_lo = b_hi + (uint32_t)p.b_half;
+#pragma unroll
+            for (int ch = 0; ch < MAX_CHUNKS; ++ch) {
+                if (!blive[ch]) continue;
+                float hi[4], lo[4];
+#pragma unroll
+                for (int e = 0; e < 4; ++e) split_tf32(vb[ch].v[e], hi[e], lo[e]);
+#pragma unroll
+                for (int e = 0; e < 4; ++e) {
+                    st_shared_f32(b_hi + boff[ch] + 16u * e, hi[e]);
+                    st_shared_f32(b_lo + boff[ch] + 16u * e, lo[e]);
+                }
+            }
             fence_proxy_async();
             mbar_arrive(full(s));
         };
         if constexpr (!TMA) {
-            F4 a0[NAU], a1[NAU], b0[NBU], b1[NBU];
+            F4 a0[2], a1[2], b0[MAX_CHUNKS], b1[MAX_CHUNKS];
             bool k0 = false, k1 = false;
             int it = 0;
             if (it < nkb) load(it, a0, b0, k0);
             for (; it < nkb; it += 2) {
                 const bool more = it + 1 < nkb;
                 if (more) load(it + 1, a1, b1, k1);
-                store(it, a0, b0, k0);
+                store(a0, b0, k0);
                 if (more) {
                     if (it + 2 < nkb) load(it + 2, a0, b0, k0);
-                    store(it + 1, a1, b1, k1);
+                    store(a1, b1, k1);
                 }
             }
         } else {
-            F4 xc[NAU], xn[NAU], va[NAU], vb[NBU];
+            auto issue = [&](int it, int j) {
+                const uint32_t dst = base + ring_off + (uint32_t)j * (uint32_t)p.slot_bytes;
+                const int q0 = q_begin + it * KP;
+                mbar_arrive_expect_tx(rfull(j), (uint32_t)p.slot_tx);
+                uint32_t seg = dst;
+                if (!UP) {
+                    tma_tile_2d(dst, &tmx, ci_tile * BLOCK_CI, q0, rfull(j));
+                    seg += X_BYTES;
+                }
+                for (int ky = 0; ky < p.KH; ++ky)
+                    tma_tile_2d(seg + (uint32_t)ky * (uint32_t)p.seg_bytes, &tmd, co0,
+                                q0 - (ky * p.dil - p.pad) * p.Wout - p.tox_max, rfull(j));
+            };
+            if (pt == 0) {
+                if (!UP) tma_prefetch_desc(&tmx);
+                tma_prefetch_desc(&tmd);
+                for (int it = 0; it < nkb && it < p.ring; ++it) issue(it, it);
+            }
+            F4 xc[2], xn[2], va[2], vb[MAX_CHUNKS];
             bool kc = false, kn = false, okx = false;
             Cursor pre = cur;
             if (UP && nkb > 0) { load_x(0, pre, xc, kc); advance(pre); }
@@ -415,14 +392,18 @@
                 mbar_wait(rfull(rj), rph);
                 ring_read(it, base + ring_off + (uint32_t)rj * (uint32_t)p.slot_bytes, va, vb, okx);
                 mbar_arrive(rempty(rj));
+                if (pt == 0 && it + p.ring < nkb) {
+                    mbar_wait(rempty(rj), rph);
+                    issue(it + p.ring, rj);
+                }
                 if (++rj == p.ring) { rj = 0; rph ^= 1; }
                 if (UP) {
-                    store(it, xc, vb, okx);
-#pragma unroll
-                    for (int ch = 0; ch < NAU; ++ch) xc[ch] = xn[ch];
+                    store(xc, vb, okx);
+#pragma unroll
+                    for (int h = 0; h < 2; ++h) xc[h] = xn[h];
                     kc = kn;
                 } else {
-                    store(it, va, vb, okx);
+                    store(va, vb, okx);
                 }
             }
         }
@@ -463,7 +444,7 @@
     const int taps = KH * KW;
     const int cg = bts_wgrad2_cg(Cout, taps);
     const long long Mq = (long long)B * Hin * Win;
-    const long long KBq = (Mq + KP - 1) / KP;
+    const long long KBq = (Mq + SPLIT_PX - 1) / SPLIT_PX;
     const long long tiles = (long long)((Cin + BLOCK_CI - 1) / BLOCK_CI) * ((Cout + cg - 1) / cg);
     const int sms = bts_num_sms();
     long long max_split = (KBq + g_w2_min_kb - 1) / g_w2_min_kb;
@@ -527,15 +508,14 @@
     p.dy = dy; p.dys = dys; p.Cout = Cout; p.Hout = Hout; p.Wout = Wout;
     p.Hin = up ? 2 * Hs : Hs; p.Win = up ? 2 * Ws : Ws;
     p.cg = bts_wgrad2_cg(Cout, taps);
-    p.nb = (p.cg + 31) / 32;
     p.part = workspace; p.splitK = splitK;
     const long long Mq = (long long)B * p.Hin * p.Win;
     if (Mq > 0x7ffffff0LL) return BTS_EINVAL;
     p.Mq = (int)Mq;
-    p.KBq = (int)((Mq + KP - 1) / KP);
-    p.kb_per_split = (p.KBq + splitK - 1) / splitK;
-    p.nchunks = (taps * p.cg + 31) / 32;
-    p.stage_bytes = 2 * A_BYTES + 2 * p.nchunks * 4 * (int)CORE_SBO;
+    const int blocks = (int)((Mq + SPLIT_PX - 1) / SPLIT_PX);
+    p.px_per_split = (blocks + splitK - 1) / splitK * SPLIT_PX;
+    p.b_half = taps * p.cg / 8 * (int)CORE_SBO;
+    p.stage_bytes = (X_BYTES + 2 * p.b_half + 127) / 128 * 128;
     p.stages = SMEM_BUDGET / p.stage_bytes;
     if (p.stages > MAX_STAGES) p.stages = MAX_STAGES;
     if (p.stages < 2) return BTS_EINVAL;
@@ -551,8 +531,8 @@
         p.segw = KP + (KW - 1) * dil;
         p.tox_max = (KW - 1) * dil - pad;
         p.seg_bytes = (p.segw * p.cg * 4 + 127) / 128 * 128;
-        p.slot_bytes = (up ? 0 : X_RAW_BYTES) + KH * p.seg_bytes;
-        p.slot_tx = (up ? 0 : X_RAW_BYTES) + KH * p.segw * p.cg * 4;
+        p.slot_bytes = (up ? 0 : X_BYTES) + KH * p.seg_bytes;
+        p.slot_tx = (up ? 0 : X_BYTES) + KH * p.segw * p.cg * 4;
         int st_try = p.stages > 3 ? 3 : p.stages;
         for (; st_try >= 2 && !tma; --st_try) {
             const int ring = (SMEM_BUDGET - st_try * p.stage_bytes) / p.slot_bytes;
```

New measurement: 75.01, median of 6. 1.08x the previous value.
